# BBischof/ESRecsys

Hardware: AMD Instinct MI355X
Metric: training pairs/sec (higher is better)
Workload: dtype f32; 1 GPU; inbatch: V=1000000 x D=128 fp32 tables, B=8192, sparse Adagrad; score_precision=auto -> f16x2, ids=uniform, parallelism=single

## Files before the change

### esrecsys_amd/csrc/esr_inbatch2h.hip

```cpp
#include "esr_inbatch_mfma.h"
#include "esr_segment.h"
#include <atomic>
#include <type_traits>
#include <time.h>

namespace esr {

typedef _Float16 f16x8 __attribute__((ext_vector_type(8)));
typedef _Float16 f16x2 __attribute__((ext_vector_type(2)));

constexpr int kHLseOff = 2 * kPlaneBytes;
constexpr int kHBufBytes = kHLseOff + 4 * 256;
constexpr float kHOptHead = 4.0f;
constexpr float kHOverflow = 60000.0f;
constexpr int kHBufs = 3;
constexpr float kHPexp = 14.0f;
constexpr float kHBoundSafe = 14.0f;
constexpr int kHScaleWords = 8;

#define H_MFMA(a, b, c) __builtin_amdgcn_mfma_f32_32x32x16_f16((a), (b), (c), 0, 0, 0)
#define H_SB() __builtin_amdgcn_sched_barrier(0)
#define H_DMA_BARRIER()                                 \
  {                                                     \
    asm volatile("s_waitcnt vmcnt(0)" ::: "memory");    \
// ... 578 lines not shown
    if (VALU_ON) pst_u += nch * 4096;                                                                     \
  }
#if defined(H_PROBE_NOMFMA)
#define H_O_ROW(PL_A, PL_P, G)                                                                            \
  _Pragma("unroll") for (int db_ = 0; db_ < 4; ++db_) {                                                   \
    acc[db_][0] += (float)ta2_[G][db_][PL_A][0] * (float)pb[PL_P][G][0];                                  \
  }
#else
#define H_O_ROW(PL_A, PL_P, G)                                                                            \
  _Pragma("unroll") for (int db_ = 0; db_ < 4; ++db_)                                                     \
    acc[db_] = H_MFMA(ta2_[G][db_][PL_A], pb[PL_P][G], acc[db_]);
#endif
#if defined(H_PROBE_PC_NOFRAG)
#define H_O_G1(F0, F1)
#else
#define H_O_G1(F0, F1) { _Pragma("unroll") for (int f_ = (F0); f_ < (F1); ++f_) trh_frag_n<1>(f_, ta2_, trc_); }
#endif
#define H_PB()                                                                                            \
  f16x8 pb[2][2];                                                                                         \
  _Pragma("unroll") for (int q_ = 0; q_ < 2; ++q_)                                                        \
    _Pragma("unroll") for (int g_ = 0; g_ < 2; ++g_) {                                                    \
      const u32x4 u_ = {pw[q_][4 * g_], pw[q_][4 * g_ + 1], pw[q_][4 * g_ + 2], pw[q_][4 * g_ + 3]};      \
      pb[q_][g_] = __builtin_bit_cast(f16x8, u_);                                                         \
    }
#define H_O_PHASE(DMA_ON, DBUF)                                                                           \
  {                                                                                                       \
    H_PB();                                                                                               \
    H_TR_WAIT();     \
    H_SB(); H_O_ROW(1, 0, 0); H_SB(); H_O_G1(0, 3); if (DMA_ON) { H_DP(0, g0, DBUF); }                    \
    H_SB(); H_O_ROW(0, 1, 0); H_SB(); H_O_G1(3, 6); if (DMA_ON) { H_DP(1, g1, DBUF); }                    \
    H_SB(); H_O_ROW(0, 0, 0); H_SB(); H_O_G1(6, 8); if (DMA_ON) { H_DP(2, g2, DBUF); }                    \
    H_TR_WAIT();                                                                                          \
    H_SB(); H_O_ROW(1, 0, 1); H_SB(); if (DMA_ON) { H_DP(3, g3, DBUF); }                                  \
    H_SB(); H_O_ROW(0, 1, 1); H_SB();                                                                     \
    H_SB(); H_O_ROW(0, 0, 1); H_SB();                                                                     \
    if (DMA_ON) H_DMA_ADVANCE();                                                                          \
  }
#define H_TR_BASES(BUF)                                                                                   \
  {                                                                                                       \
    const uint32_t slot_ = (uint32_t)((BUF) - lds);                                                       \
    _Pragma("unroll") for (int db_ = 0; db_ < 4; ++db_) { trc_[db_][0] = trb_[db_][0] + slot_; trc_[db_][1] = trb_[db_][1] + slot_; } \
  }
#define H_TR_SETUP()                                                                                      \
  const int tr_a = (lane & 15) >> 2;                                                                      \
  const int tr_e = (2 * ((lane >> 4) & 1)) + ((lane & 3) >> 1), tr_low = (lane & 1) * 8;                  \
  const int tr_row0 = (4 * h + tr_a) * 256, tr_row1 = (4 * h + 8 + tr_a) * 256;                           \
  const int tr_l0 = ((tr_e ^ (h & 3)) << 4) | tr_low, tr_l1 = ((tr_e ^ ((h + 2) & 3)) << 4) | tr_low;     \
  uint32_t trb_[4][2], trc_[4][2];                                                                        \
  _Pragma("unroll") for (int db = 0; db < 4; ++db) {                                                      \
    trb_[db][0] = (uint32_t)(uintptr_t)(__attribute__((address_space(3))) const char*)lds + tr_row0 + (((db ^ tr_a) << 6) | tr_l0); \
    trb_[db][1] = (uint32_t)(uintptr_t)(__attribute__((address_space(3))) const char*)lds + tr_row1 + (((db ^ tr_a) << 6) | tr_l1); \
  }

template <int KIND>
__global__ ESR_NO_PK __launch_bounds__(256) __attribute__((amdgpu_waves_per_eu(2, 2))) void inbatch2h_q_kernel(const _Float16* __restrict__ Xr, const _Float16* __restrict__ Yr,
                                                         int64_t B, int nsplit, float sl2_in,
                                                         const float* __restrict__ sc, const float* __restrict__ ref,
                                                         int nsplit_ref, const float* __restrict__ diag, int mode,
                                                         int* __restrict__ flags, float* __restrict__ part_m,
                                                         float* __restrict__ part_O, float* __restrict__ part_l,
                                                         float* __restrict__ Pmat) {
  __shared__ __attribute__((aligned(16))) char lds[kHBufs * kHBufBytes];
  if (KIND == 1 && flags[blockIdx.x] == 0) return;
  H_TIMING_DECL();
  int t = threadIdx.x, lane = t & 63;
  const int w = __builtin_amdgcn_readfirstlane(t >> 6);
  int j = lane & 31, h = lane >> 5;
  H_TR_SETUP();
  const uint32_t lds32 = (uint32_t)(uintptr_t)(__attribute__((address_space(3))) const char*)lds;
  (void)lds32;
  const int ob = blockIdx.x / nsplit, split = blockIdx.x % nsplit;
  const int64_t xrow = (int64_t)ob * k3Owned + w * 32 + j;
  const int nc = (int)(B / k3Chunk) / nsplit;
  const int64_t c0 = (int64_t)split * nc;
  const int64_t nch = B / 32;
  const float sl2 = sl2_in * sc[0];

  char* pst_u = nullptr;
  const uint32_t pst_v = (uint32_t)((((j >> 3) * 16) + ((2 * h + ((j >> 2) & 1)) * 4) + (j & 3)) * 16);
#if defined(H_PROBE_Q_NOSTORE)
#define H_P_ST(M, V0, V1, V2, V3)
#else
#define H_P_ST(M, V0, V1, V2, V3) \
  __builtin_nontemporal_store(u32x4{(V0), (V1), (V2), (V3)}, reinterpret_cast<u32x4*>(pst_u + (M) * 1024 + pst_v))
#endif

  f32x16 acc[4];
  f32x2 l2 = {0.f, 0.f};
  int dpos = 0;
  const char* const baseY = reinterpret_cast<const char*>(Yr);
  uint32_t g0 = 0, g1 = 0, g2 = 0, g3 = 0;
  f16x8 bx[2][8];
#pragma unroll
  for (int p = 0; p < 2; ++p)
#pragma unroll
    for (int s = 0; s < 8; ++s)
      bx[p][s] = *reinterpret_cast<const f16x8*>(Xr + ((int64_t)p * B + xrow) * k3D + 16 * s + 8 * h);
  f32x16 sa;
  float p[16];
  uint32_t pw[2][8];
  f16x8 ta2_[2][4][2];
  float emax = 0.f;
  float refv = -INFINITY;
  const f32x2 sl2v = {sl2, sl2};
  f32x2 nrefv = {0.f, 0.f};
  auto sweep = [&](auto fix_tag) __attribute__((always_inline)) {
  constexpr bool fix = decltype(fix_tag)::value;
  pst_u = reinterpret_cast<char*>(Pmat) + (c0 * nch + (xrow >> 5)) * 4096;
#pragma unroll
  for (int db = 0; db < 4; ++db)
#pragma unroll
    for (int r = 0; r < 16; ++r) acc[db][r] = 0.f;
  l2 = f32x2{0.f, 0.f};
  dpos = 0;
  g0 = dmah_off0<0>(B, c0, t); g1 = dmah_off0<1>(B, c0, t); g2 = dmah_off0<2>(B, c0, t); g3 = dmah_off0<3>(B, c0, t);
  emax = 0.f;
  refv = -INFINITY;
#pragma unroll
  for (int r = 0; r < 16; ++r) p[r] = 0.f;
  if (fix) {
    float m = -INFINITY;
    for (int c = 0; c < nc; ++c) {
      H_DMA_CHUNK(lds);
      H_DMA_BARRIER();
      H_S_PHASE(lds, sa, false);
#pragma unroll
      for (int r = 0; r < 16; ++r) m = fmaxf(m, sa[r] * sl2);
      __syncthreads();
    }
    refv = fmaxf(m, __shfl_xor(m, 32, 64)) - kHPexp;
  }
  const bool sample = !fix && mode == 1 && c0 != 0;
  if (sample) {
    char* sbuf = lds + 2 * kHBufBytes;
    H_DP(0, dmah_off0<0>(B, 0, t), sbuf); H_DP(1, dmah_off0<1>(B, 0, t), sbuf);
    H_DP(2, dmah_off0<2>(B, 0, t), sbuf); H_DP(3, dmah_off0<3>(B, 0, t), sbuf);
  }
  H_DMA_CHUNK(lds);
  if (nc > 1) H_DMA_CHUNK(lds + kHBufBytes);
  if (!fix && mode == 0) {
    float rv[8];
#pragma unroll
    for (int s = 0; s < 8; ++s) rv[s] = s < nsplit_ref ? ref[(int64_t)s * B + xrow] : -INFINITY;
    refv = rv[0];
#pragma unroll
    for (int s = 1; s < 8; ++s) refv = fmaxf(refv, rv[s]);
  }
  const float dref = (!fix && mode == 1) ? diag[xrow] * sl2_in : -INFINITY;
  H_DMA_BARRIER();

  float msample = dref;
  if (sample) {
    H_S_PHASE(lds + 2 * kHBufBytes, sa, false);
#pragma unroll
    for (int r = 0; r < 16; ++r) msample = fmaxf(msample, sa[r] * sl2);
  }
  H_S_PHASE(lds, sa, false);
#pragma unroll
  for (int r = 0; r < 16; ++r) p[r] = sa[r];
  if (!fix && mode == 1) {
    float m = msample;
    if (!sample) {
#pragma unroll
      for (int r = 0; r < 16; ++r) m = fmaxf(m, sa[r] * sl2);
    }
    refv = fmaxf(m, __shfl_xor(m, 32, 64)) - kHOptHead;
  }
  if (h == 0) part_m[(int64_t)split * B + xrow] = refv;
  nrefv = f32x2{-refv, -refv};

  H_TIMING_START();
  int cur = 0;
  for (int it = 0; it + 2 < nc; ++it) {
    const int nxt = cur == kHBufs - 1 ? 0 : cur + 1;
    const int nn = nxt == kHBufs - 1 ? 0 : nxt + 1;
    H_TICK(tk0);
    H_DMA_BARRIER();
    H_TICK(tk1);
    const char* buf = lds + cur * kHBufBytes;
    const char* nbuf = lds + nxt * kHBufBytes;
    char* dbuf = lds + nn * kHBufBytes;
    H_TR_BASES(buf);
    H_S_PHASE(nbuf, sa, true);
    H_TICK(tk2);
#pragma unroll
    for (int r = 0; r < 16; ++r) p[r] = sa[r];
    H_O_PHASE(true, dbuf);
    H_TICK(tk3);
    H_TIMING_ACC();
    cur = nxt;
  }
  if (nc >= 2) {
    const int nxt = cur == kHBufs - 1 ? 0 : cur + 1;
    H_DMA_BARRIER();
    const char* buf = lds + cur * kHBufBytes;
    const char* nbuf = lds + nxt * kHBufBytes;
    H_TR_BASES(buf);
    H_S_PHASE(nbuf, sa, true);
#pragma unroll
    for (int r = 0; r < 16; ++r) p[r] = sa[r];
    H_O_PHASE(false, lds);
    cur = nxt;
  }
  {
    H_DMA_BARRIER();
    const char* buf = lds + cur * kHBufBytes;
    H_TR_BASES(buf);
#pragma unroll
    for (int f = 0; f < 8; ++f) trh_frag_n<0>(f, ta2_, trc_);
#pragma unroll
    for (int s = 0; s < 8; ++s) {
      const f32x2 arg = f32x2{p[2 * s], p[2 * s + 1]} * sl2v + nrefv;
      const float e0 = __builtin_amdgcn_exp2f(arg[0]);
      const float e1 = __builtin_amdgcn_exp2f(arg[1]);
      l2 += f32x2{e0, e1};
      emax = fmaxf(emax, fmaxf(e0, e1));
      const f16x2 pa = pk_f16(e0, e1);
      const f16x2 pq = pk_f16(resid_lo(e0, pa), resid_hi(e1, pa));
      pw[0][s] = __builtin_bit_cast(uint32_t, pa);
      pw[1][s] = __builtin_bit_cast(uint32_t, pq);
    }
#pragma unroll
    for (int m2 = 0; m2 < 2; ++m2)
#pragma unroll
      for (int pl = 0; pl < 2; ++pl) {
        H_P_ST(2 * m2 + pl, pw[pl][4 * m2], pw[pl][4 * m2 + 1], pw[pl][4 * m2 + 2], pw[pl][4 * m2 + 3]);
      }
    H_O_PHASE(false, lds);
  }
  };
  if (KIND == 1) {
    sweep(std::true_type{});
  } else {
    sweep(std::false_type{});
    if (KIND == 2 && mode != 0 && __syncthreads_or((mode == 2 || !(emax <= kHOverflow)) ? 1 : 0)) {
      asm volatile("" : "+v"(t), "+v"(lane), "+v"(j), "+v"(h));
      sweep(std::true_type{});
    }
  }
#undef H_P_ST
  H_TIMING_WRITE(H_TIMING_Q);
  float* orow = part_O + ((int64_t)split * B + xrow) * k3D;
#pragma unroll
  for (int db = 0; db < 4; ++db)
#pragma unroll
    for (int q = 0; q < 4; ++q)
      *reinterpret_cast<float4*>(orow + 32 * db + 8 * q + 4 * h) =
          make_float4(acc[db][4 * q], acc[db][4 * q + 1], acc[db][4 * q + 2], acc[db][4 * q + 3]);
  const float l = l2[0] + l2[1];
  const float ltot = l + __shfl_xor(l, 32, 64);
  if (h == 0) part_l[(int64_t)split * B + xrow] = ltot;
  if (KIND == 0 && (mode == 2 || !(emax <= kHOverflow))) flags[blockIdx.x] = 1;
}

template <int K>
__device__ __forceinline__ uint32_t dmah8_off0(int64_t B, int64_t chunk, int t) {
  const int row = t >> 4, seg = (t & 15) ^ swz16(row);
  return (uint32_t)((((int64_t)K * B + chunk * 32 + row) * k3D + seg * 8) * 2);
}
constexpr int kH1Waves = 8, kH1Owned = 32 * kH1Waves;
constexpr int kH1BufBytes = kPlaneBytes + kH1Waves * 256;
#define H1_DP(K, G, BUF) dmah_piece<K>(baseY, G, (BUF), w)
#define H1_DMA_REF(BUF)                                                                                   \
  __builtin_amdgcn_global_load_lds((gptr_t)(ref + (c0 + dpos) * 32 + (lane & 31)),                        \
                                   (lptr_t)((BUF) + kPlaneBytes + w * 256), 4, 0, 0)
#define H1_DMA_ADVANCE()                                                                   \
  {                                                                                        \
    const uint32_t step_ = (dpos + 1 == nc) ? (uint32_t)(8192 - nc * 8192) : 8192u;        \
    dpos = (dpos + 1 == nc) ? 0 : dpos + 1;                                                \
    g0 += step_;                                                                           \
  }
#define H1_DMA_CHUNK(BUF) { if (!QSIDE) { H1_DMA_REF(BUF); } H1_DP(0, g0, BUF); H1_DMA_ADVANCE(); }
#define H1_LOAD_REFS(BUF)                                                                                 \
  if (!QSIDE) {                                                                                           \
    f16x8 raw_[4];                                                                                        \
    _Pragma("unroll") for (int m_ = 0; m_ < 4; ++m_)                                                      \
      raw_[m_] = lds_b128<0>(lds32 + (uint32_t)((BUF) - lds) + (uint32_t)(kPlaneBytes + w * 256 + (8 * m_ + 4 * h) * 4)); \
    H_TR_WAIT();                                                                                          \
    _Pragma("unroll") for (int m_ = 0; m_ < 4; ++m_) {                                                    \
      const float4 lv_ = __builtin_bit_cast(float4, raw_[m_]);                                            \
      rf[4 * m_] = kHPexp - lv_.x; rf[4 * m_ + 1] = kHPexp - lv_.y;                                       \
      rf[4 * m_ + 2] = kHPexp - lv_.z; rf[4 * m_ + 3] = kHPexp - lv_.w;                                   \
    }                                                                                                     \
  }
#define H1_EXP_PAIR(S, PN)                                                                                \
  {                                                                                                       \
    const float a0_ = fma_s(p[2 * (S)], sl2, QSIDE ? nref1 : rf[2 * (S)]);                                \
    const float a1_ = fma_s(p[2 * (S) + 1], sl2, QSIDE ? nref1 : rf[2 * (S) + 1]);                        \
    const float e0_ = __builtin_amdgcn_exp2f(a0_), e1_ = __builtin_amdgcn_exp2f(a1_);                     \
    const f16x2 pa_ = pk_f16(e0_, e1_);                                                                   \
    if (QSIDE) { sum_max(l2a, l2b, emax, e0_, e1_); }                                                     \
    const f16x2 pq_ = pk_f16(resid_lo(e0_, pa_), resid_hi(e1_, pa_));                                     \
    PN[0][(S)] = __builtin_bit_cast(uint32_t, pa_);                                                       \
    PN[1][(S)] = __builtin_bit_cast(uint32_t, pq_);                                                       \
  }
#define H1_S_PHASE(NBUF, SA)                                                                              \
  {                                                                                                       \
    _Pragma("unroll") for (int r_ = 0; r_ < 16; ++r_) SA[r_] = 0.f;                                       \
    const uint32_t ap32_ = lds32 + (uint32_t)((NBUF) - lds) + (uint32_t)(j * 256);                        \
    const int sw_ = swz16(j);                                                                             \
    f16x8 af_[8];                                                                                         \
    _Pragma("unroll") for (int s_ = 0; s_ < 8; ++s_)                                                      \
      af_[s_] = lds_b128<0>(ap32_ + (uint32_t)(((2 * s_ + h) ^ sw_) << 4));                               \
    _Pragma("unroll") for (int s_ = 0; s_ < 8; ++s_) {                                                    \
// ... 350 lines not shown
#define CT_PROBE_NOP 0
#endif
#if defined(CT_PROBE_NO_DMA)
#define CT_PROBE_NOY 1
#else
#define CT_PROBE_NOY 0
#endif
#ifndef CT_P_IN_LOAD
#define CT_P_IN_LOAD 4
#endif
constexpr int kCtRing = 3;
constexpr int kCtYSlot = 2 * kPlaneBytes + 8 * 256;
constexpr int kCtPOff = kCtRing * kCtYSlot;
constexpr int kCtPSlot = 4096 + 64;
constexpr int kCtPWave = kCtRing * kCtPSlot;
constexpr int kCtLds = kCtPOff + 8 * kCtPWave;
constexpr int kCtOwned = 256;
constexpr float kCtLive = 0.0625f;
#ifndef H_P_LOAD_AUX
#define H_P_LOAD_AUX 2
#endif

template <int G, int F, int SLOTOFF, class TA>
__device__ __forceinline__ void ct_frag(TA& ta, const uint32_t (&tb)[4][2]) {
  constexpr int PL = (F / 4 + 1) % 2, DB = F % 4, OFF = SLOTOFF + PL * kPlaneBytes + 16 * G * 256;
  const s16x4 lo = tr_read<OFF>(tb[DB][0]), hi = tr_read<OFF>(tb[DB][1]);
  const s16x8 both = {lo[0], lo[1], lo[2], lo[3], hi[0], hi[1], hi[2], hi[3]};
  ta[G][DB][PL] = __builtin_bit_cast(f16x8, both);
}
template <int G, int SLOTOFF, class TA>
__device__ __forceinline__ void ct_frag_n(int f, TA& ta, const uint32_t (&tb)[4][2]) {
  switch (f) {
    case 0: ct_frag<G, 0, SLOTOFF>(ta, tb); break;
    case 1: ct_frag<G, 1, SLOTOFF>(ta, tb); break;
    case 2: ct_frag<G, 2, SLOTOFF>(ta, tb); break;
    case 3: ct_frag<G, 3, SLOTOFF>(ta, tb); break;
    case 4: ct_frag<G, 4, SLOTOFF>(ta, tb); break;
    case 5: ct_frag<G, 5, SLOTOFF>(ta, tb); break;
    case 6: ct_frag<G, 6, SLOTOFF>(ta, tb); break;
    default: ct_frag<G, 7, SLOTOFF>(ta, tb); break;
  }
}
template <int PL, int G, int SLOTOFF>
__device__ __forceinline__ f16x8 ct_pfrag(uint32_t pbase) {
  constexpr int OFF = SLOTOFF + PL * 1024 + G * 512;
  const s16x4 lo = tr_read<OFF>(pbase), hi = tr_read<OFF + 256>(pbase);
  const s16x8 both = {lo[0], lo[1], lo[2], lo[3], hi[0], hi[1], hi[2], hi[3]};
  return __builtin_bit_cast(f16x8, both);
}

__global__ ESR_NO_PK __launch_bounds__(512) void inbatch2h_pct_kernel(
    const _Float16* __restrict__ Yt, const _Float16* __restrict__ Yh, int64_t B, int nsplit,
    const float* __restrict__ fac, int nc_q, const char* __restrict__ Pt, float cexp,
    const int* __restrict__ cflags, int force_general, float* __restrict__ part_O) {
  constexpr int kLdsBytes = kCtLds > 8 * kTileLdsBytes ? kCtLds : 8 * kTileLdsBytes;
  __shared__ __attribute__((aligned(16))) char lds[kLdsBytes];
  const int t = threadIdx.x, lane = t & 63;
  const int w = __builtin_amdgcn_readfirstlane(t >> 6);
  const int j = lane & 31, h = lane >> 5;
  (void)j;
  H_TR_SETUP();
  (void)trc_;
  const int ob = blockIdx.x / nsplit, split = blockIdx.x % nsplit;
  const int64_t wrow = (int64_t)ob * kCtOwned + w * 32;
  const bool live = wrow < B;
  const int nc = (int)(B / k3Chunk) / nsplit;
  const int64_t c0 = (int64_t)split * nc;
  const int64_t nch = B / 32;
  const int64_t jt = live ? (wrow >> 5) : 0;
  bool general = force_general != 0;
  if (!general) {
    const int s_lo = (int)(((int64_t)ob * (kCtOwned / 32)) / nc_q);
    const int s_hi = (int)(min((int64_t)ob * (kCtOwned / 32) + (kCtOwned / 32 - 1), nch - 1) / nc_q);
    for (int sq = s_lo; sq <= s_hi; ++sq) general = general || cflags[sq] != 0;
  }
  const float* ref = fac + (int64_t)(jt / nc_q) * B;
  const char* const pw_base = Pt + (jt * nch + c0) * 4096;
  const uint32_t lds32 = (uint32_t)(uintptr_t)(__attribute__((address_space(3))) const char*)lds;
  uint32_t p_off[4];
#pragma unroll
  for (int g4 = 0; g4 < 4; ++g4) p_off[g4] = (uint32_t)(g4 * 1024 + lane * 16);
  const uint32_t pbase = lds32 + (uint32_t)(kCtPOff + w * kCtPWave + ((lane >> 4) & 1) * (2048 + 64) +
                                            (2 * ((lane & 3) >> 1) + h) * 64 + tr_a * 16 + (lane & 1) * 8);
  const uint32_t rbase = lds32 + (uint32_t)(2 * kPlaneBytes + w * 256 + 16 * h);

  f32x16 acc[4];
#pragma unroll
  for (int db = 0; db < 4; ++db)
#pragma unroll
    for (int r = 0; r < 16; ++r) acc[db][r] = 0.f;
  f16x8 ta2_[2][4][2];
  f16x8 pb[2][2];
  float rf[16];
#pragma unroll
  for (int r = 0; r < 16; ++r) rf[r] = 0.f;

  auto sweep = [&](auto gen_tag) __attribute__((always_inline)) {
    constexpr bool GEN = decltype(gen_tag)::value;
    constexpr int kWaitTop = CT_PROBE_NOP ? (CT_PROBE_NOY ? 0 : 2) : 4 + (GEN ? 3 : 2) + 4;
    const char* const baseY = reinterpret_cast<const char*>(GEN ? Yh : Yt);
    const char* const dummy = reinterpret_cast<const char*>(Yh);
    int dpos = 0;
    uint32_t g0 = dmah8_off0<0>(B, c0, t), g1 = dmah8_off0<1>(B, c0, t);
    const int wq = w & 3;
#define CT_DMA_Y_PIECE(SLOT, I)                                                                           \
  if (!CT_PROBE_NOY) {                                                                                    \
    if ((I) == 0)                                                                                         \
      __builtin_amdgcn_global_load_lds((gptr_t)(baseY + g0), (lptr_t)(lds + (SLOT) * kCtYSlot + w * 1024), 16, 0, 0); \
    if ((I) == 1)                                                                                         \
      __builtin_amdgcn_global_load_lds((gptr_t)(baseY + g1),                                              \
                                       (lptr_t)(lds + (SLOT) * kCtYSlot + kPlaneBytes + w * 1024), 16, 0, 0); \
    if ((I) == 2) {                                                                                       \
      if (GEN)                                                                                            \
        __builtin_amdgcn_global_load_lds((gptr_t)(ref + (c0 + dpos) * 32 + (lane & 31)),                 \
                                         (lptr_t)(lds + (SLOT) * kCtYSlot + 2 * kPlaneBytes + w * 256), 4, 0, 0); \
      const uint32_t step_ = (dpos + 1 == nc) ? (uint32_t)(8192 - nc * 8192) : 8192u;                     \
      dpos = (dpos + 1 == nc) ? 0 : dpos + 1;                                                             \
      g0 += step_; g1 += step_;                                                                           \
    }                                                                                                     \
  }
#define CT_DMA_Y(SLOT) { CT_DMA_Y_PIECE(SLOT, 0); CT_DMA_Y_PIECE(SLOT, 1); CT_DMA_Y_PIECE(SLOT, 2); }
#define CT_DMA_P_PIECE(SLOT, CH, G4)                                                                      \
  if (!CT_PROBE_NOP) {                                                                                    \
    const char* src_ = (!CT_PROBE_DUMMY && (CH) < nc) ? pw_base + (int64_t)(CH) * 4096 : dummy;           \
    __builtin_amdgcn_global_load_lds((gptr_t)(src_ + p_off[G4]),                                          \
                                     (lptr_t)(lds + kCtPOff + w * kCtPWave + (SLOT) * kCtPSlot + (G4) * 1024 +  \
                                              ((G4) >> 1) * 64), 16, 0,                                   \
// ... 129 lines not shown
    sweep(std::false_type{});
    const float ce = cexp;
#pragma unroll
    for (int db = 0; db < 4; ++db)
#pragma unroll
      for (int r = 0; r < 16; ++r) acc[db][r] *= ce;
  }
  asm volatile("s_waitcnt vmcnt(0)" ::: "memory");
  __syncthreads();
  if (live) store_tile_via_lds<true>(lds + w * kTileLdsBytes, acc, part_O + ((int64_t)split * B + wrow) * k3D, lane);
}

__global__ __launch_bounds__(256) void fac2h_kernel(int64_t B, int nsplit, const float* __restrict__ part_m,
                                                   const float* __restrict__ part_l, float invl_scale,
                                                   float* __restrict__ fac, float* __restrict__ lse2 = nullptr,
                                                   float* __restrict__ lse_nat = nullptr) {
  const int64_t row = (int64_t)blockIdx.x * 256 + threadIdx.x;
  if (row >= B) return;
  float pm[8], pl[8];
#pragma unroll
  for (int s = 0; s < 8; ++s) {
    pm[s] = -INFINITY; pl[s] = 0.f;
    if (s < nsplit) {
      pm[s] = part_m[(int64_t)s * B + row];
      pl[s] = part_l[(int64_t)s * B + row];
    }
  }
  float M = pm[0], L = 0.f;
  float wt[8];
#pragma unroll
  for (int s = 1; s < 8; ++s) M = fmaxf(M, pm[s]);
#pragma unroll
  for (int s = 0; s < 8; ++s) {
    wt[s] = pm[s] == M ? 1.f : __builtin_amdgcn_exp2f(pm[s] - M);
    L = __fmaf_rn(pl[s], wt[s], L);
  }
  const float invL1 = __fdiv_rn(1.0f, L);
#pragma unroll
  for (int s = 0; s < 8; ++s)
    if (s < nsplit) fac[(int64_t)s * B + row] = __fmul_rn(__fmul_rn(invL1, invl_scale), wt[s]);
  if (lse2) {
    const float l2v = __fadd_rn(M, __builtin_amdgcn_logf(L));
    lse2[row] = l2v;
    if (lse_nat) lse_nat[row] = l2v * k3Ln2;
  }
}

constexpr int kCtExpShift = 11;
__global__ __launch_bounds__(256) void facscale2h_kernel(RowSrc X, int64_t B, int nsplit,
                                                        const float* __restrict__ part_m,
                                                        const float* __restrict__ part_l, float invl_scale,
                                                        const float* __restrict__ sc, float* __restrict__ fac,
                                                        float* __restrict__ lse2, float* __restrict__ lse_nat,
                                                        _Float16* __restrict__ Yt, int* __restrict__ cflags) {
  const int t = threadIdx.x, chunk = blockIdx.x;
  const int row = t >> 3, sl = t & 7, d0 = sl * 16;
  const int64_t grow = (int64_t)chunk * 32 + row;
  float v[16];
  {
    const int64_t r = X.idx ? (int64_t)X.idx[grow] : grow;
    RowSrc Y0 = X;
    Y0.idx = nullptr;
#pragma unroll
    for (int q = 0; q < 4; ++q) {
      const float4 f = rowsrc_load4(Y0, r, d0 + 4 * q);
      v[4 * q] = f.x; v[4 * q + 1] = f.y; v[4 * q + 2] = f.z; v[4 * q + 3] = f.w;
    }
  }
  const float pm_l = sl < nsplit ? part_m[(int64_t)sl * B + grow] : -INFINITY;
  const float pl_l = sl < nsplit ? part_l[(int64_t)sl * B + grow] : 0.f;
  float pm[8], pl[8];
  const int lane0 = (t & 63) & ~7;
#pragma unroll
  for (int s = 0; s < 8; ++s) {
    pm[s] = __shfl(pm_l, lane0 + s, 64);
    pl[s] = __shfl(pl_l, lane0 + s, 64);
  }
  float M = pm[0], L = 0.f;
  float wt[8];
#pragma unroll
  for (int s = 1; s < 8; ++s) M = fmaxf(M, pm[s]);
#pragma unroll
  for (int s = 0; s < 8; ++s) {
    wt[s] = pm[s] == M ? 1.f : __builtin_amdgcn_exp2f(pm[s] - M);
    L = __fmaf_rn(pl[s], wt[s], L);
  }
  const float invL1 = __fdiv_rn(1.0f, L);
  const float f1 = __fmul_rn(invL1, invl_scale);
  float wmine = 1.f;
#pragma unroll
  for (int s = 0; s < 8; ++s) wmine = s == sl ? wt[s] : wmine;
  const float fs = __fmul_rn(f1, wmine);
  if (sl < nsplit) {
    fac[(int64_t)sl * B + grow] = fs;
    if (fs != f1) cflags[sl] = 1;
  }
  if (sl == 0 && lse2) {
    const float l2v = __fadd_rn(M, __builtin_amdgcn_logf(L));
    lse2[grow] = l2v;
    if (lse_nat) lse_nat[grow] = l2v * k3Ln2;
  }
  const float mul = sc[3] * ldexpf(1.f, -kCtExpShift);
  float m = 0.f;
  f16x8 p[2][2];
#pragma unroll
  for (int e = 0; e < 16; ++e) {
    const float xs = __fmul_rn(v[e], f1) * mul;
    m = fmaxf(m, fabsf(xs));
    const _Float16 a = (_Float16)xs;
    const _Float16 b = (_Float16)(xs - (float)a);
    p[0][e >> 3][e & 7] = a;
    p[1][e >> 3][e & 7] = b;
  }
  m = fmaxf(m, __shfl_xor(m, 1, 64));
  m = fmaxf(m, __shfl_xor(m, 2, 64));
  m = fmaxf(m, __shfl_xor(m, 4, 64));
  if (sl < nsplit && (!(m < 60000.f) || (f1 != 0.f && m < kCtLive))) cflags[sl] = 1;
#pragma unroll
  for (int pl2 = 0; pl2 < 2; ++pl2) {
    f16x8* dst = reinterpret_cast<f16x8*>(Yt + ((int64_t)pl2 * B + grow) * k3D + d0);
    dst[0] = p[pl2][0];
    dst[1] = p[pl2][1];
  }
}

struct InbatchHWs {
  _Float16 *Qh, *Ch;
  float *part_O, *part_O2, *fac_side, *Qcopy, *Ccopy, *part_m, *part_mr, *part_l, *lse2, *fac, *Pmat, *nrm, *amax, *sc, *diag;
  int* flags;
  unsigned long long* loss_acc;
  unsigned long long* ent;
  _Float16* Qt;
  unsigned* czero;
  int* cflags;
};
constexpr int64_t kHMaxB = 16384;

static size_t inbatch2h_ws_layout(int64_t B, char* base, InbatchHWs* ws) {
  size_t off = 0;
  auto take = [&](size_t bytes) {
    char* p = base ? base + off : nullptr;
    off += align_up(bytes, 256);
    return p;
  };
  const size_t planes = (size_t)2 * B * k3D * 2;
  InbatchHWs w;
  w.Qh = (_Float16*)take(planes);
  w.Ch = (_Float16*)take(planes);
  w.part_O = (float*)take((size_t)8 * B * k3D * 4);
  w.part_O2 = (float*)take((size_t)8 * B * k3D * 4);
  w.fac_side = (float*)take((size_t)8 * B * 4);
  w.Qcopy = (float*)take((size_t)B * k3D * 4);
  w.Ccopy = (float*)take((size_t)B * k3D * 4);
  w.part_m = (float*)take((size_t)8 * B * 4);
  w.part_mr = (float*)take((size_t)8 * B * 4);
  w.part_l = (float*)take((size_t)8 * B * 4);
  w.lse2 = (float*)take((size_t)B * 4);
  w.fac = (float*)take((size_t)8 * B * 4);
  w.diag = (float*)take((size_t)B * 4);
  w.flags = (int*)take((size_t)8 * (B / k3Owned) * sizeof(int));
  w.Pmat = (float*)take((size_t)B * B * 4);
  w.loss_acc = (unsigned long long*)take(sizeof(unsigned long long) * 16 * (1 + kLossWords));
  w.nrm = (float*)take((size_t)2 * (B / k3Chunk) * 4 * sizeof(float));
  w.amax = (float*)take((size_t)2 * (B / k3Chunk) * sizeof(float));
  w.sc = (float*)take(kHScaleWords * sizeof(float));
  w.ent = (unsigned long long*)take((size_t)(B / k3Chunk + 1) * sizeof(unsigned long long));
  w.Qt = (_Float16*)take(planes);
  w.czero = (unsigned*)take(16 * sizeof(unsigned));
  w.cflags = reinterpret_cast<int*>(w.czero ? w.czero + 8 : nullptr);
  if (ws) *ws = w;
// ... 53 lines not shown
static int inbatch2h_run(const char* who, RowSrc Qs, RowSrc Cs, const int32_t* gq_rows, const int32_t* gc_rows, int64_t B,
                         int D, float scale, float regularization, float batch_size, float* loss, float* lse,
                         float* gQ, float* gC, void* workspace, size_t workspace_bytes, esr_stream_t stream,
                         hipStream_t side = nullptr, const InbatchUpdate* upd = nullptr) {
  if (!(B > 0 && B % k3Owned == 0 && B <= kHMaxB)) {
    set_error("%s: B=%lld must be a positive multiple of 128, at most %lld (larger batches: the bf16x3 entry point)",
              who, (long long)B, (long long)kHMaxB);
    return ESR_EINVAL;
  }
  if (!(D > 0 && D <= k3D && D % 4 == 0)) {
    set_error("%s: D=%d not supported (a multiple of 4, at most 128; wider rows: the f32 entry point)", who, D);
    return ESR_EINVAL;
  }
  if (!(Qs.base && Cs.base && loss && gQ && gC)) {
    set_error("%s: null pointer", who);
    return ESR_EINVAL;
  }
  if (batch_size == 0.f) {
    set_error("%s: batch_size must be non-zero", who);
    return ESR_EINVAL;
  }
  if ((((uintptr_t)Qs.base | (uintptr_t)Cs.base | (uintptr_t)gQ | (uintptr_t)gC) & 15) != 0) {
    set_error("%s: matrices must be 16-byte aligned", who);
    return ESR_EINVAL;
  }
  if (!workspace || workspace_bytes < esr_inbatch2h_workspace_bytes(B, D) || ((uintptr_t)workspace & 15)) {
    set_error("%s: workspace %zu bytes < %zu required (or misaligned)", who, workspace_bytes,
              esr_inbatch2h_workspace_bytes(B, D));
    return ESR_EWORKSPACE;
  }
  hipStream_t st = as_stream(stream);
  InbatchHWs ws;
  inbatch2h_ws_layout(B, (char*)workspace, &ws);
  const float inv_bs = 1.0f / batch_size, sl2 = scale * k3Log2e;
  const int nchunks = (int)(B / k3Chunk);
  const char* qcs = getenv("ESR_IB2H_Q_PER_CU");
  const int nsplit_q = inbatch2h_nsplit(B, qcs ? std::max(1, atoi(qcs)) : 2);
  const int pc_blocks = (int)cdiv(B, kCtOwned);
  int nsplit_c = 1;
  for (int sp = 1; sp <= 8; ++sp)
    if (nchunks % sp == 0 && pc_blocks * sp <= 320) nsplit_c = sp;
  const int grid_c = pc_blocks * nsplit_c;
  const int grid_q = (int)(B / k3Owned) * nsplit_q;
  const int mgrid = (int)std::min<int64_t>(k3MergeBlocks, cdiv(B, kBlock / 32));
  const char* refe = getenv("ESR_IB2H_REF");
  const int mode = (refe && refe[0] == 'r' && refe[1] == 'o') ? 0 : ((refe && refe[0] == 'r' && refe[1] == 'e') ? 2 : 1);
  const char* fe = getenv("ESR_IB2H_FUSED");
  const bool fused = !(fe && fe[0] == '0') && mode != 0;
  int nsplit_r = 1;
  hipEvent_t ev_fork = nullptr, ev_join = nullptr;
  const char* b16e = getenv("ESR_IB2H_BF16");
  const bool one_plane = fused && ((Qs.bf16 && Cs.bf16 && !(b16e && b16e[0] == 't')) || (b16e && b16e[0] == 'f'));
  const bool overlapped = fused && !one_plane && side != nullptr && side != st && inbatch_events(&ev_fork, &ev_join);
  const char* mue = getenv("ESR_IB2H_MERGE_UPDATE");
  const bool merge_upd = fused && !overlapped && upd != nullptr && upd->skip_long && D == k3D && Qs.ld == k3D &&
                         Cs.ld == k3D && !(mue && mue[0] == '0');
  auto merging_update = [&](int nsplit_of_c, const float* part_O_of_c) -> int {
    InbatchMergeArgs a;
    a.part_O[0] = ws.part_O; a.part_O[1] = part_O_of_c;
    a.nsplit[0] = nsplit_q; a.nsplit[1] = nsplit_of_c;
    a.oscale[0] = ws.sc + 1; a.oscale[1] = ws.sc + 2;
    a.partner[0] = ws.Ccopy; a.partner[1] = ws.Qcopy;
    a.part_m = ws.part_m; a.part_l = ws.part_l;
    a.B = B;
    a.scale = scale; a.lam = regularization; a.inv_bs = inv_bs;
    a.loss_acc = ws.loss_acc; a.loss_scale = 1.0 / (double)batch_size; a.loss_out = loss;
    a.zero_words = ws.ent; a.nzero = nchunks + 1;
    return inbatch_merge_update(upd->tables, upd->accums, upd->row_offsets, upd->dtype, upd->sorted_vids, upd->perm, a,
                                upd->lr, upd->eps, st);
  };
  if (fused) {
    static std::atomic<unsigned long long> call_seq{0};
    static const unsigned long long seed =
        (unsigned long long)(uintptr_t)&call_seq ^ (unsigned long long)time(nullptr) * 0x9E3779B97F4A7C15ull;
    unsigned long long z = seed + 0x9E3779B97F4A7C15ull * (call_seq.fetch_add(1) + 1);
    z = (z ^ (z >> 30)) * 0xBF58476D1CE4E5B9ull;
    z = (z ^ (z >> 27)) * 0x94D049BB133111EBull;
    const unsigned long long token = ((z ^ (z >> 31)) >> 16) | 1ull;
    const char* tle = getenv("ESR_IB2H_POLL");
    const int two_level = (tle && tle[0] == 'f') ? 0 : 1;
    ESR_KT("prepsplit2h_kernel", st,
           hipLaunchKernelGGL(prepsplit2h_kernel, dim3(nchunks), dim3(256), 0, st, Qs, Cs, B, ws.Qh, ws.Ch, ws.ent, token,
                              ws.diag, ws.nrm, ws.sc, ws.loss_acc, ws.flags, grid_q, (overlapped || merge_upd) ? ws.Qcopy : (float*)nullptr,
                              (overlapped || merge_upd) ? ws.Ccopy : (float*)nullptr, ws.czero, two_level));
    if (one_plane) {
      const int blocks1 = (int)cdiv(B, kH1Owned);
      int nsplit_1 = 1;
      for (int sp = 1; sp <= 8; ++sp)
        if (nchunks % sp == 0 && blocks1 * sp <= 320) nsplit_1 = sp;
      const int nsplit_q = nsplit_1, grid_q = blocks1 * nsplit_1;
      const char* dbg1h = getenv("ESR_IB1H_DBG");
      if (dbg1h && dbg1h[0] == '1') {
        hipLaunchKernelGGL((inbatch1h_kernel<true, 1>), dim3(grid_q), dim3(512), 0, st, (const _Float16*)ws.Qh,
                           (const _Float16*)ws.Ch, B, nsplit_q, sl2, (const float*)ws.sc, (const float*)ws.diag,
                           (const float*)nullptr, mode, ws.part_m, ws.part_O, ws.part_l);
      } else
      ESR_KT("inbatch1h_kernel_q", st,
             hipLaunchKernelGGL((inbatch1h_kernel<true>), dim3(grid_q), dim3(512), 0, st, (const _Float16*)ws.Qh,
                                (const _Float16*)ws.Ch, B, nsplit_q, sl2, (const float*)ws.sc, (const float*)ws.diag,
                                (const float*)nullptr, mode, ws.part_m, ws.part_O, ws.part_l));
      if (merge_upd) {
        ESR_KT("fac2h_kernel", st,
               hipLaunchKernelGGL(fac2h_kernel, dim3((unsigned)cdiv(B, 256)), dim3(256), 0, st, B, nsplit_q,
                                  (const float*)ws.part_m, (const float*)ws.part_l, ldexpf(1.f, (int)kHPexp), ws.fac,
                                  ws.lse2, lse));
      } else
      ESR_KT("inbatch3_merge_kernel_q", st,
             hipLaunchKernelGGL((inbatch3_merge_kernel<true>), dim3(mgrid), dim3(kBlock), 0, st, Qs, Cs, gq_rows, B,
                                nsplit_q, (const float*)ws.part_O, (const float*)ws.part_m, (const float*)ws.part_l, scale,
                                regularization, inv_bs, ws.lse2, lse, gQ, ws.loss_acc, 1.0 / (double)batch_size, loss,
                                (float*)nullptr, (const float*)(ws.sc + 1), ldexpf(1.f, (int)kHPexp), ws.fac));
      float* const part_O_1c = merge_upd ? ws.part_O2 : ws.part_O;
      if (dbg1h && (dbg1h[0] == '1' || dbg1h[0] == '2')) {
        hipLaunchKernelGGL((inbatch1h_kernel<false, 1>), dim3(grid_q), dim3(512), 0, st, (const _Float16*)ws.Ch,
                           (const _Float16*)ws.Qh, B, nsplit_q, sl2, (const float*)ws.sc, (const float*)nullptr,
                           (const float*)ws.lse2, mode, (float*)nullptr, part_O_1c, (float*)nullptr);
      } else
      ESR_KT("inbatch1h_kernel_c", st,
             hipLaunchKernelGGL((inbatch1h_kernel<false>), dim3(grid_q), dim3(512), 0, st, (const _Float16*)ws.Ch,
                                (const _Float16*)ws.Qh, B, nsplit_q, sl2, (const float*)ws.sc, (const float*)nullptr,
                                (const float*)ws.lse2, mode, (float*)nullptr, part_O_1c, (float*)nullptr));
      if (merge_upd) return merging_update(nsplit_q, part_O_1c);
      ESR_KT("inbatch3_merge_kernel_c", st,
             hipLaunchKernelGGL((inbatch3_merge_kernel<false>), dim3(mgrid), dim3(kBlock), 0, st, Cs, Qs, gc_rows, B,
                                nsplit_q, (const float*)ws.part_O, (const float*)ws.part_m, (const float*)ws.part_l, scale,
                                regularization, inv_bs, ws.lse2, (float*)nullptr, gC, ws.loss_acc,
                                1.0 / (double)batch_size, loss, (float*)nullptr, (const float*)(ws.sc + 2), 1.0f,
                                (float*)nullptr, ws.ent, nchunks + 1));
      if (upd) {
        const int rc = sparse_adagrad_range(upd->tables, upd->accums, upd->row_offsets, 2, upd->dtype, D, upd->sorted_vids,
                                            upd->perm, 2 * B, upd->grad_rows, upd->lr, upd->eps, upd->skip_long, st);
        if (rc != ESR_OK) return rc;
      }
      return check_launch(who);
    }
    ESR_KT("inbatch2h_q_kernel", st,
           hipLaunchKernelGGL((inbatch2h_q_kernel<2>), dim3(grid_q), dim3(256), 0, st, (const _Float16*)ws.Qh,
                              (const _Float16*)ws.Ch, B, nsplit_q, sl2, (const float*)ws.sc, (const float*)ws.part_mr, 1,
                              (const float*)ws.diag, mode, ws.flags, ws.part_m, ws.part_O, ws.part_l, ws.Pmat));
  } else {
  ESR_KT("prep2h_kernel", st, hipLaunchKernelGGL(prep2h_kernel, dim3(nchunks), dim3(256), 0, st, Qs, Cs, ws.amax, ws.diag));
  ESR_KT("split2h_kernel", st,
         hipLaunchKernelGGL(split2h_kernel, dim3(nchunks, 2), dim3(256), 0, st, Qs, Cs, B, ws.Qh, ws.Ch,
                            (const float*)ws.amax, ws.nrm, ws.sc, ws.loss_acc, ws.flags, grid_q));
  if (mode == 0) {
    const int rm_blocks = (int)cdiv(B, kHRmOwned);
    for (int sp = 1; sp <= 8; ++sp)
      if (nchunks % sp == 0 && rm_blocks * sp <= 320) nsplit_r = sp;
    ESR_KT("rowmax2h_kernel", st,
           hipLaunchKernelGGL(rowmax2h_kernel, dim3(rm_blocks * nsplit_r), dim3(256), 0, st, (const _Float16*)ws.Qh,
                              (const _Float16*)ws.Ch, B, nsplit_r, sl2, (const float*)ws.nrm, (const float*)ws.sc,
                              ws.part_mr));
  }
  {
    ESR_KT("inbatch2h_q_kernel", st,
           hipLaunchKernelGGL((inbatch2h_q_kernel<0>), dim3(grid_q), dim3(256), 0, st, (const _Float16*)ws.Qh,
                              (const _Float16*)ws.Ch, B, nsplit_q, sl2, (const float*)ws.sc, (const float*)ws.part_mr,
                              nsplit_r, (const float*)ws.diag, mode, ws.flags, ws.part_m, ws.part_O, ws.part_l, ws.Pmat));
    if (mode != 0)
      ESR_KT("inbatch2h_q_kernel_redo", st,
             hipLaunchKernelGGL((inbatch2h_q_kernel<1>), dim3(grid_q), dim3(256), 0, st, (const _Float16*)ws.Qh,
                                (const _Float16*)ws.Ch, B, nsplit_q, sl2, (const float*)ws.sc, (const float*)ws.part_mr,
                                nsplit_r, (const float*)ws.diag, mode, ws.flags, ws.part_m, ws.part_O, ws.part_l, ws.Pmat));
  }
  }
  hipStream_t st_q = overlapped ? side : st;
  float* const part_O_c = (overlapped || merge_upd) ? ws.part_O2 : ws.part_O;
  const RowSrc Qm = overlapped ? RowSrc{ws.Qcopy, nullptr, 0, Qs.ld} : Qs;
  const RowSrc Cm = overlapped ? RowSrc{ws.Ccopy, nullptr, 0, Cs.ld} : Cs;
  const int nc_q = nchunks / nsplit_q;
  const char* pcm = getenv("ESR_IB2H_PC");
  const int force_general = (!fused || (pcm && pcm[0] == 'g')) ? 1 : 0;
  if (overlapped) {
    if (hipEventRecord(ev_fork, st) != hipSuccess || hipStreamWaitEvent(side, ev_fork, 0) != hipSuccess) {
      set_error("%s: could not fork the side stream", who);
      return ESR_ELAUNCH;
    }
  }
  if (!force_general)
    ESR_KT("facscale2h_kernel", st,
           hipLaunchKernelGGL(facscale2h_kernel, dim3(nchunks), dim3(256), 0, st,
                              (overlapped || merge_upd) ? RowSrc{ws.Qcopy, nullptr, 0, Qs.ld} : Qs, B, nsplit_q,
                              (const float*)ws.part_m, (const float*)ws.part_l, ldexpf(1.f, (int)kHPexp),
                              (const float*)ws.sc, ws.fac, merge_upd ? ws.lse2 : (float*)nullptr,
                              merge_upd ? lse : (float*)nullptr, ws.Qt, ws.cflags));
  else if (overlapped || merge_upd)
    ESR_KT("fac2h_kernel", st,
           hipLaunchKernelGGL(fac2h_kernel, dim3((unsigned)cdiv(B, 256)), dim3(256), 0, st, B, nsplit_q,
                              (const float*)ws.part_m, (const float*)ws.part_l, ldexpf(1.f, (int)kHPexp), ws.fac,
                              merge_upd ? ws.lse2 : (float*)nullptr, merge_upd ? lse : (float*)nullptr));
  if (!merge_upd)
  ESR_KT("inbatch3_merge_kernel_q", st_q,
         hipLaunchKernelGGL((inbatch3_merge_kernel<true>), dim3(mgrid), dim3(kBlock), 0, st_q, Qm, Cm, gq_rows, B, nsplit_q,
                            (const float*)ws.part_O, (const float*)ws.part_m, (const float*)ws.part_l, scale,
                            regularization, inv_bs, ws.lse2, lse, gQ, ws.loss_acc, 1.0 / (double)batch_size, loss,
                            (float*)nullptr, (const float*)(ws.sc + 1), ldexpf(1.f, (int)kHPexp),
                            overlapped ? ws.fac_side : ws.fac));
  if (overlapped) {
    if (upd) {
      const int rc = sparse_adagrad_range(upd->tables, upd->accums, upd->row_offsets, 2, upd->dtype, D, upd->sorted_vids,
                                          upd->perm, B, upd->grad_rows, upd->lr, upd->eps, upd->skip_long, side);
      if (rc != ESR_OK) return rc;
    }
    if (hipEventRecord(ev_join, side) != hipSuccess) {
      set_error("%s: could not record the join event", who);
      return ESR_ELAUNCH;
    }
  }
  ESR_KT("inbatch2h_pct_kernel", st,
         hipLaunchKernelGGL(inbatch2h_pct_kernel, dim3(grid_c), dim3(512), 0, st, (const _Float16*)ws.Qt,
                            (const _Float16*)ws.Qh, B, nsplit_c, (const float*)ws.fac, nc_q, (const char*)ws.Pmat,
                            ldexpf(1.f, kCtExpShift), (const int*)ws.cflags, force_general, part_O_c));
  if (merge_upd) return merging_update(nsplit_c, part_O_c);
  ESR_KT("inbatch3_merge_kernel_c", st,
         hipLaunchKernelGGL((inbatch3_merge_kernel<false>), dim3(mgrid), dim3(kBlock), 0, st, Cm, Qm, gc_rows, B, nsplit_c,
                            (const float*)part_O_c, (const float*)ws.part_m, (const float*)ws.part_l, scale,
                            regularization, inv_bs, ws.lse2, (float*)nullptr, gC, ws.loss_acc,
                            1.0 / (double)batch_size, loss, (float*)nullptr, (const float*)(ws.sc + 2), 1.0f,
                            (float*)nullptr, fused ? ws.ent : (unsigned long long*)nullptr, nchunks + 1));
  if (upd) {
    const int64_t off = overlapped ? B : 0;
    const int rc = sparse_adagrad_range(upd->tables, upd->accums, upd->row_offsets, 2, upd->dtype, D,
                                        upd->sorted_vids + off, upd->perm + off, 2 * B - off, upd->grad_rows, upd->lr,
                                        upd->eps, upd->skip_long, st);
    if (rc != ESR_OK) return rc;
  }
  if (overlapped && hipStreamWaitEvent(st, ev_join, 0) != hipSuccess) {
    set_error("%s: could not join the side stream", who);
    return ESR_ELAUNCH;
  }
  return check_launch(who);
}

int esr_inbatch_softmax_fwd_bwd_f16x2(const float* Q, const float* C, int64_t B, int D, float scale,
                                      float regularization, float batch_size, float* loss, float* lse, float* gQ,
                                      float* gC, void* workspace, size_t workspace_bytes, esr_stream_t stream) {
  TraceScope trace_scope_("esr_inbatch_softmax_fwd_bwd_f16x2");
  return inbatch2h_run("esr_inbatch_softmax_fwd_bwd_f16x2", RowSrc{Q, nullptr, 0, D}, RowSrc{C, nullptr, 0, D}, nullptr,
                       nullptr, B, D, scale, regularization, batch_size, loss, lse, gQ, gC, workspace, workspace_bytes,
                       stream);
}

int esr_inbatch_towers_fwd_bwd_f16x2(const void* query_table, int64_t Vq, const void* cand_table, int64_t Vc, int dtype,
                                     int D, const int32_t* query_ids, const int32_t* cand_ids, const int32_t* gq_rows,
                                     const int32_t* gc_rows, int64_t B, float scale, float regularization,
                                     float batch_size, float* loss, float* lse, float* gQ, float* gC, void* workspace,
                                     size_t workspace_bytes, esr_stream_t stream) {
  TraceScope trace_scope_("esr_inbatch_towers_fwd_bwd_f16x2");
  ESR_REQUIRE(Vq > 0 && Vc > 0 && query_ids && cand_ids, "esr_inbatch_towers_fwd_bwd_f16x2: bad tables / ids");
  ESR_REQUIRE(dtype == ESR_F32 || dtype == ESR_BF16, "esr_inbatch_towers_fwd_bwd_f16x2: bad dtype %d", dtype);
  return inbatch2h_run("esr_inbatch_towers_fwd_bwd_f16x2", RowSrc{query_table, query_ids, dtype == ESR_BF16, D},
                       RowSrc{cand_table, cand_ids, dtype == ESR_BF16, D}, gq_rows, gc_rows, B, D, scale, regularization,
                       batch_size, loss, lse, gQ, gC, workspace, workspace_bytes, stream);
}

int esr_inbatch2h_pass_c_forms(const void* workspace, size_t workspace_bytes, int64_t B, int32_t* forms,
                               esr_stream_t stream) {
  ESR_REQUIRE(workspace && forms && B > 0 && B % k3Owned == 0 && B <= kHMaxB &&
                  workspace_bytes >= esr_inbatch2h_workspace_bytes(B, k3D),
              "esr_inbatch2h_pass_c_forms: bad workspace / B");
  InbatchHWs ws;
  inbatch2h_ws_layout(B, (char*)const_cast<void*>(workspace), &ws);
  if (hipMemcpyAsync(forms, ws.cflags, 8 * sizeof(int32_t), hipMemcpyDeviceToDevice, as_stream(stream)) != hipSuccess) {
    set_error("esr_inbatch2h_pass_c_forms: copy failed");
    return ESR_ELAUNCH;
// ... 85 lines not shown
```

Baseline: 37.58 million pairs/s.

## Pair adjacent Q-kernel splits in one block and reduce partials through LDS

Result: no change. 37.89 million pairs/s, median of 6 (+0.8%).

```diff
diff --git a/esrecsys_amd/csrc/esr_inbatch2h.hip b/esrecsys_amd/csrc/esr_inbatch2h.hip
--- a/esrecsys_amd/csrc/esr_inbatch2h.hip
+++ b/esrecsys_amd/csrc/esr_inbatch2h.hip
@@ -654,24 +654,29 @@
     trb_[db][1] = (uint32_t)(uintptr_t)(__attribute__((address_space(3))) const char*)lds + tr_row1 + (((db ^ tr_a) << 6) | tr_l1); \
   }
 
-template <int KIND>
-__global__ ESR_NO_PK __launch_bounds__(256) __attribute__((amdgpu_waves_per_eu(2, 2))) void inbatch2h_q_kernel(const _Float16* __restrict__ Xr, const _Float16* __restrict__ Yr,
+template <int KIND, bool PAIR = false>
+__global__ ESR_NO_PK __launch_bounds__(PAIR ? 512 : 256) __attribute__((amdgpu_waves_per_eu(2, 2))) void inbatch2h_q_kernel(const _Float16* __restrict__ Xr, const _Float16* __restrict__ Yr,
                                                          int64_t B, int nsplit, float sl2_in,
                                                          const float* __restrict__ sc, const float* __restrict__ ref,
                                                          int nsplit_ref, const float* __restrict__ diag, int mode,
                                                          int* __restrict__ flags, float* __restrict__ part_m,
                                                          float* __restrict__ part_O, float* __restrict__ part_l,
                                                          float* __restrict__ Pmat) {
-  __shared__ __attribute__((aligned(16))) char lds[kHBufs * kHBufBytes];
+  static_assert(!PAIR || KIND == 2, "the paired form redoes itself in the kernel");
+  __shared__ __attribute__((aligned(16))) char lds_all[(PAIR ? 2 : 1) * kHBufs * kHBufBytes];
   if (KIND == 1 && flags[blockIdx.x] == 0) return;
   H_TIMING_DECL();
-  int t = threadIdx.x, lane = t & 63;
-  const int w = __builtin_amdgcn_readfirstlane(t >> 6);
+  const int wall = __builtin_amdgcn_readfirstlane((int)threadIdx.x >> 6);
+  const int half = PAIR ? wall >> 2 : 0, w = PAIR ? (wall & 3) : wall;
+  char* const lds = lds_all + half * (kHBufs * kHBufBytes);
+  int t = PAIR ? ((int)threadIdx.x & 255) : (int)threadIdx.x, lane = t & 63;
   int j = lane & 31, h = lane >> 5;
   H_TR_SETUP();
   const uint32_t lds32 = (uint32_t)(uintptr_t)(__attribute__((address_space(3))) const char*)lds;
   (void)lds32;
-  const int ob = blockIdx.x / nsplit, split = blockIdx.x % nsplit;
+  const int nslot = PAIR ? nsplit / 2 : nsplit;
+  const int ob = blockIdx.x / nslot, slot = blockIdx.x % nslot;
+  const int split = PAIR ? 2 * slot + half : slot;
   const int64_t xrow = (int64_t)ob * k3Owned + w * 32 + j;
   const int nc = (int)(B / k3Chunk) / nsplit;
   const int64_t c0 = (int64_t)split * nc;
@@ -730,7 +735,15 @@
       for (int r = 0; r < 16; ++r) m = fmaxf(m, sa[r] * sl2);
       __syncthreads();
     }
-    refv = fmaxf(m, __shfl_xor(m, 32, 64)) - kHPexp;
+    m = fmaxf(m, __shfl_xor(m, 32, 64));
+    if (PAIR) {
+      float* const xm = reinterpret_cast<float*>(lds_all);
+      if (h == 0) xm[half * k3Owned + w * 32 + j] = m;
+      __syncthreads();
+      m = fmaxf(m, xm[(half ^ 1) * k3Owned + w * 32 + j]);
+      __syncthreads();
+    }
+    refv = m - kHPexp;
   }
   const bool sample = !fix && mode == 1 && c0 != 0;
   if (sample) {
@@ -768,7 +781,7 @@
     }
     refv = fmaxf(m, __shfl_xor(m, 32, 64)) - kHOptHead;
   }
-  if (h == 0) part_m[(int64_t)split * B + xrow] = refv;
+  if (h == 0 && half == 0) part_m[(int64_t)slot * B + xrow] = refv;
   nrefv = f32x2{-refv, -refv};
 
   H_TIMING_START();
@@ -842,16 +855,40 @@
   }
 #undef H_P_ST
   H_TIMING_WRITE(H_TIMING_Q);
-  float* orow = part_O + ((int64_t)split * B + xrow) * k3D;
+  const float l = l2[0] + l2[1];
+  float ltot = l + __shfl_xor(l, 32, 64);
+  if constexpr (PAIR) {
+    float4* const xo = reinterpret_cast<float4*>(lds_all);
+    float* const xl = reinterpret_cast<float*>(lds_all + 16 * 256 * sizeof(float4));
+    static_assert(16 * 256 * sizeof(float4) + k3Owned * sizeof(float) <= sizeof(lds_all), "hand-over outgrows the rings");
+    __syncthreads();
+    if (half == 1) {
+#pragma unroll
+      for (int db = 0; db < 4; ++db)
+#pragma unroll
+        for (int q = 0; q < 4; ++q)
+          xo[(4 * db + q) * 256 + t] = make_float4(acc[db][4 * q], acc[db][4 * q + 1], acc[db][4 * q + 2], acc[db][4 * q + 3]);
+      if (h == 0) xl[w * 32 + j] = ltot;
+    }
+    __syncthreads();
+    if (half == 1) return;
+#pragma unroll
+    for (int db = 0; db < 4; ++db)
+#pragma unroll
+      for (int q = 0; q < 4; ++q) {
+        const float4 v = xo[(4 * db + q) * 256 + t];
+        acc[db][4 * q] += v.x; acc[db][4 * q + 1] += v.y; acc[db][4 * q + 2] += v.z; acc[db][4 * q + 3] += v.w;
+      }
+    ltot += xl[w * 32 + j];
+  }
+  float* orow = part_O + ((int64_t)slot * B + xrow) * k3D;
 #pragma unroll
   for (int db = 0; db < 4; ++db)
 #pragma unroll
     for (int q = 0; q < 4; ++q)
       *reinterpret_cast<float4*>(orow + 32 * db + 8 * q + 4 * h) =
           make_float4(acc[db][4 * q], acc[db][4 * q + 1], acc[db][4 * q + 2], acc[db][4 * q + 3]);
-  const float l = l2[0] + l2[1];
-  const float ltot = l + __shfl_xor(l, 32, 64);
-  if (h == 0) part_l[(int64_t)split * B + xrow] = ltot;
+  if (h == 0) part_l[(int64_t)slot * B + xrow] = ltot;
   if (KIND == 0 && (mode == 2 || !(emax <= kHOverflow))) flags[blockIdx.x] = 1;
 }
 
@@ -1308,7 +1345,7 @@
 __global__ ESR_NO_PK __launch_bounds__(512) void inbatch2h_pct_kernel(
     const _Float16* __restrict__ Yt, const _Float16* __restrict__ Yh, int64_t B, int nsplit,
     const float* __restrict__ fac, int nc_q, const char* __restrict__ Pt, float cexp,
-    const int* __restrict__ cflags, int force_general, float* __restrict__ part_O) {
+    const int* __restrict__ cflags, int cf_rep, int force_general, float* __restrict__ part_O) {
   constexpr int kLdsBytes = kCtLds > 8 * kTileLdsBytes ? kCtLds : 8 * kTileLdsBytes;
   __shared__ __attribute__((aligned(16))) char lds[kLdsBytes];
   const int t = threadIdx.x, lane = t & 63;
@@ -1328,7 +1365,7 @@
   if (!general) {
     const int s_lo = (int)(((int64_t)ob * (kCtOwned / 32)) / nc_q);
     const int s_hi = (int)(min((int64_t)ob * (kCtOwned / 32) + (kCtOwned / 32 - 1), nch - 1) / nc_q);
-    for (int sq = s_lo; sq <= s_hi; ++sq) general = general || cflags[sq] != 0;
+    for (int sq = s_lo; sq <= s_hi; ++sq) general = general || cflags[sq * cf_rep] != 0;
   }
   const float* ref = fac + (int64_t)(jt / nc_q) * B;
   const char* const pw_base = Pt + (jt * nch + c0) * 4096;
@@ -1564,7 +1601,8 @@
                                                         const float* __restrict__ part_l, float invl_scale,
                                                         const float* __restrict__ sc, float* __restrict__ fac,
                                                         float* __restrict__ lse2, float* __restrict__ lse_nat,
-                                                        _Float16* __restrict__ Yt, int* __restrict__ cflags) {
+                                                        _Float16* __restrict__ Yt, int* __restrict__ cflags,
+                                                        int cf_rep) {
   const int t = threadIdx.x, chunk = blockIdx.x;
   const int row = t >> 3, sl = t & 7, d0 = sl * 16;
   const int64_t grow = (int64_t)chunk * 32 + row;
@@ -1605,7 +1643,8 @@
   const float fs = __fmul_rn(f1, wmine);
   if (sl < nsplit) {
     fac[(int64_t)sl * B + grow] = fs;
-    if (fs != f1) cflags[sl] = 1;
+    if (fs != f1)
+      for (int c = 0; c < cf_rep; ++c) cflags[sl * cf_rep + c] = 1;
   }
   if (sl == 0 && lse2) {
     const float l2v = __fadd_rn(M, __builtin_amdgcn_logf(L));
@@ -1627,7 +1666,8 @@
   m = fmaxf(m, __shfl_xor(m, 1, 64));
   m = fmaxf(m, __shfl_xor(m, 2, 64));
   m = fmaxf(m, __shfl_xor(m, 4, 64));
-  if (sl < nsplit && (!(m < 60000.f) || (f1 != 0.f && m < kCtLive))) cflags[sl] = 1;
+  if (sl < nsplit && (!(m < 60000.f) || (f1 != 0.f && m < kCtLive)))
+    for (int c = 0; c < cf_rep; ++c) cflags[sl * cf_rep + c] = 1;
 #pragma unroll
   for (int pl2 = 0; pl2 < 2; ++pl2) {
     f16x8* dst = reinterpret_cast<f16x8*>(Yt + ((int64_t)pl2 * B + grow) * k3D + d0);
@@ -1787,13 +1827,17 @@
   const char* b16e = getenv("ESR_IB2H_BF16");
   const bool one_plane = fused && ((Qs.bf16 && Cs.bf16 && !(b16e && b16e[0] == 't')) || (b16e && b16e[0] == 'f'));
   const bool overlapped = fused && !one_plane && side != nullptr && side != st && inbatch_events(&ev_fork, &ev_join);
+  const char* pre = getenv("ESR_IB2H_PAIR");
+  const bool pair_q = fused && !one_plane && !(Qs.bf16 && Cs.bf16) && nsplit_q % 2 == 0 && !(pre && pre[0] == '0');
+  const int nslot_q = pair_q ? nsplit_q / 2 : nsplit_q;
+  const int cf_rep = pair_q ? 2 : 1;
   const char* mue = getenv("ESR_IB2H_MERGE_UPDATE");
   const bool merge_upd = fused && !overlapped && upd != nullptr && upd->skip_long && D == k3D && Qs.ld == k3D &&
                          Cs.ld == k3D && !(mue && mue[0] == '0');
   auto merging_update = [&](int nsplit_of_c, const float* part_O_of_c) -> int {
     InbatchMergeArgs a;
     a.part_O[0] = ws.part_O; a.part_O[1] = part_O_of_c;
-    a.nsplit[0] = nsplit_q; a.nsplit[1] = nsplit_of_c;
+    a.nsplit[0] = nslot_q; a.nsplit[1] = nsplit_of_c;
     a.oscale[0] = ws.sc + 1; a.oscale[1] = ws.sc + 2;
     a.partner[0] = ws.Ccopy; a.partner[1] = ws.Qcopy;
     a.part_m = ws.part_m; a.part_l = ws.part_l;
@@ -1869,6 +1913,12 @@
       }
       return check_launch(who);
     }
+    if (pair_q)
+      ESR_KT("inbatch2h_q_kernel", st,
+             hipLaunchKernelGGL((inbatch2h_q_kernel<2, true>), dim3(grid_q / 2), dim3(512), 0, st, (const _Float16*)ws.Qh,
+                                (const _Float16*)ws.Ch, B, nsplit_q, sl2, (const float*)ws.sc, (const float*)ws.part_mr, 1,
+                                (const float*)ws.diag, mode, ws.flags, ws.part_m, ws.part_O, ws.part_l, ws.Pmat));
+    else
     ESR_KT("inbatch2h_q_kernel", st,
            hipLaunchKernelGGL((inbatch2h_q_kernel<2>), dim3(grid_q), dim3(256), 0, st, (const _Float16*)ws.Qh,
                               (const _Float16*)ws.Ch, B, nsplit_q, sl2, (const float*)ws.sc, (const float*)ws.part_mr, 1,
@@ -1903,7 +1953,7 @@
   float* const part_O_c = (overlapped || merge_upd) ? ws.part_O2 : ws.part_O;
   const RowSrc Qm = overlapped ? RowSrc{ws.Qcopy, nullptr, 0, Qs.ld} : Qs;
   const RowSrc Cm = overlapped ? RowSrc{ws.Ccopy, nullptr, 0, Cs.ld} : Cs;
-  const int nc_q = nchunks / nsplit_q;
+  const int nc_q = nchunks / nslot_q;
   const char* pcm = getenv("ESR_IB2H_PC");
   const int force_general = (!fused || (pcm && pcm[0] == 'g')) ? 1 : 0;
   if (overlapped) {
@@ -1915,18 +1965,18 @@
   if (!force_general)
     ESR_KT("facscale2h_kernel", st,
            hipLaunchKernelGGL(facscale2h_kernel, dim3(nchunks), dim3(256), 0, st,
-                              (overlapped || merge_upd) ? RowSrc{ws.Qcopy, nullptr, 0, Qs.ld} : Qs, B, nsplit_q,
+                              (overlapped || merge_upd) ? RowSrc{ws.Qcopy, nullptr, 0, Qs.ld} : Qs, B, nslot_q,
                               (const float*)ws.part_m, (const float*)ws.part_l, ldexpf(1.f, (int)kHPexp),
                               (const float*)ws.sc, ws.fac, merge_upd ? ws.lse2 : (float*)nullptr,
-                              merge_upd ? lse : (float*)nullptr, ws.Qt, ws.cflags));
+                              merge_upd ? lse : (float*)nullptr, ws.Qt, ws.cflags, cf_rep));
   else if (overlapped || merge_upd)
     ESR_KT("fac2h_kernel", st,
-           hipLaunchKernelGGL(fac2h_kernel, dim3((unsigned)cdiv(B, 256)), dim3(256), 0, st, B, nsplit_q,
+           hipLaunchKernelGGL(fac2h_kernel, dim3((unsigned)cdiv(B, 256)), dim3(256), 0, st, B, nslot_q,
                               (const float*)ws.part_m, (const float*)ws.part_l, ldexpf(1.f, (int)kHPexp), ws.fac,
                               merge_upd ? ws.lse2 : (float*)nullptr, merge_upd ? lse : (float*)nullptr));
   if (!merge_upd)
   ESR_KT("inbatch3_merge_kernel_q", st_q,
-         hipLaunchKernelGGL((inbatch3_merge_kernel<true>), dim3(mgrid), dim3(kBlock), 0, st_q, Qm, Cm, gq_rows, B, nsplit_q,
+         hipLaunchKernelGGL((inbatch3_merge_kernel<true>), dim3(mgrid), dim3(kBlock), 0, st_q, Qm, Cm, gq_rows, B, nslot_q,
                             (const float*)ws.part_O, (const float*)ws.part_m, (const float*)ws.part_l, scale,
                             regularization, inv_bs, ws.lse2, lse, gQ, ws.loss_acc, 1.0 / (double)batch_size, loss,
                             (float*)nullptr, (const float*)(ws.sc + 1), ldexpf(1.f, (int)kHPexp),
@@ -1945,7 +1995,7 @@
   ESR_KT("inbatch2h_pct_kernel", st,
          hipLaunchKernelGGL(inbatch2h_pct_kernel, dim3(grid_c), dim3(512), 0, st, (const _Float16*)ws.Qt,
                             (const _Float16*)ws.Qh, B, nsplit_c, (const float*)ws.fac, nc_q, (const char*)ws.Pmat,
-                            ldexpf(1.f, kCtExpShift), (const int*)ws.cflags, force_general, part_O_c));
+                            ldexpf(1.f, kCtExpShift), (const int*)ws.cflags, cf_rep, force_general, part_O_c));
   if (merge_upd) return merging_update(nsplit_c, part_O_c);
   ESR_KT("inbatch3_merge_kernel_c", st,
          hipLaunchKernelGGL((inbatch3_merge_kernel<false>), dim3(mgrid), dim3(kBlock), 0, st, Cm, Qm, gc_rows, B, nsplit_c,
```
